# SZU-Speech/Acoustic-Echo-Cancellation

Measured on NVIDIA B200. Metric: audio_seconds_per_second_stage1_aec, higher is better.
Workload: dtype f32

## Files before the change

acoustic_echo_cancellation_b200/csrc/fft_warp.cuh:

```cuda
#pragma once
#include <cuda_runtime.h>

namespace aec {

__device__ __forceinline__ float2 cadd(float2 a, float2 b) { return make_float2(a.x + b.x, a.y + b.y); }
__device__ __forceinline__ float2 csub(float2 a, float2 b) { return make_float2(a.x - b.x, a.y - b.y); }
__device__ __forceinline__ float2 cmul(float2 a, float2 b) {
    return make_float2(fmaf(-a.y, b.y, a.x * b.x), fmaf(a.y, b.x, a.x * b.y));
}
__device__ __forceinline__ float2 cmulc(float2 a, float2 b) {
    return make_float2(fmaf(a.y, b.y, a.x * b.x), fmaf(a.y, b.x, -(a.x * b.y)));
}
__device__ __forceinline__ float2 cfma(float2 a, float2 b, float2 acc) {
    return make_float2(fmaf(-a.y, b.y, fmaf(a.x, b.x, acc.x)), fmaf(a.y, b.x, fmaf(a.x, b.y, acc.y)));
}
__device__ __forceinline__ float2 cfmac(float2 a, float2 b, float2 acc) {
    return make_float2(fmaf(a.y, b.y, fmaf(a.x, b.x, acc.x)), fmaf(-a.y, b.x, fmaf(a.x, b.y, acc.y)));
}

template <bool INV>
__device__ __forceinline__ void radix4(float2& a, float2& b, float2& c, float2& d) {
    const float2 s0 = cadd(a, c), d0 = csub(a, c);
    const float2 s1 = cadd(b, d), d1 = csub(b, d);
    const float2 r = INV ? make_float2(-d1.y, d1.x) : make_float2(d1.y, -d1.x);
    a = cadd(s0, s1);
    c = csub(s0, s1);
    b = cadd(d0, r);
    d = csub(d0, r);
}

template <int M, bool INV>
__device__ __forceinline__ float2 mul_w16(float2 v) {
    constexpr float C1 = 0.92387953251128673848f;
    constexpr float S1 = 0.38268343236508978178f;
    constexpr float R2 = 0.70710678118654752440f;
    if constexpr (M == 0) return v;
    if constexpr (M == 4) return INV ? make_float2(-v.y, v.x) : make_float2(v.y, -v.x);
    if constexpr (M == 2) {
        return INV ? make_float2(R2 * (v.x - v.y), R2 * (v.x + v.y))
                   : make_float2(R2 * (v.x + v.y), R2 * (v.y - v.x));
    }
    if constexpr (M == 6) {
        return INV ? make_float2(-R2 * (v.x + v.y), R2 * (v.x - v.y))
                   : make_float2(R2 * (v.y - v.x), -R2 * (v.x + v.y));
    }
    constexpr float cr = (M == 1) ? C1 : (M == 3) ? S1 :  -C1;
    constexpr float cif = (M == 1) ? -S1 : (M == 3) ? -C1 :  S1;
    constexpr float ci = INV ? -cif : cif;
    return make_float2(fmaf(-v.y, ci, v.x * cr), fmaf(v.y, cr, v.x * ci));
}

__host__ __device__ constexpr int fft16_index(int p) { return (p >> 2) + 4 * (p & 3); }

template <bool INV>
__device__ __forceinline__ void fft16(float2 (&v)[16]) {
#pragma unroll
    for (int j2 = 0; j2 < 4; ++j2) radix4<INV>(v[j2], v[4 + j2], v[8 + j2], v[12 + j2]);
    v[5] = mul_w16<1, INV>(v[5]);
    v[6] = mul_w16<2, INV>(v[6]);
    v[7] = mul_w16<3, INV>(v[7]);
    v[9] = mul_w16<2, INV>(v[9]);
    v[10] = mul_w16<4, INV>(v[10]);
    v[11] = mul_w16<6, INV>(v[11]);
    v[13] = mul_w16<3, INV>(v[13]);
    v[14] = mul_w16<6, INV>(v[14]);
    v[15] = mul_w16<9, INV>(v[15]);
#pragma unroll
    for (int q1 = 0; q1 < 4; ++q1) radix4<INV>(v[4 * q1], v[4 * q1 + 1], v[4 * q1 + 2], v[4 * q1 + 3]);
}

constexpr int kTilePitch = 272;

template <bool INV>
__device__ __forceinline__ void fft256_halfwarp(float2 (&v)[16], float2* tile, const float2* __restrict__ tw,
                                                int h) {
    fft16<INV>(v);
    float2* row = tile + h * 17;
    const float2* twh = tw + h;
#pragma unroll
    for (int p = 0; p < 16; ++p) {
        const int q = fft16_index(p);
        float2 x = v[p];
        if (q != 0) {
            const float2 w = __ldg(twh + q * 16);
            x = INV ? cmulc(x, w) : cmul(x, w);
        }
        row[q] = x;
    }
    __syncwarp();
    const float2* col = tile + h;
#pragma unroll
    for (int l = 0; l < 16; ++l) v[l] = col[l * 17];
    __syncwarp();
    fft16<INV>(v);
}

struct TwiddleRegs {
    float2 w1, w2, w4, w8;
};

template <bool INV>
__device__ __forceinline__ void fft256_halfwarp_regs(float2 (&v)[16], float2* tile, const TwiddleRegs& t, int h) {
    fft16<INV>(v);
    float2* row = tile + h * 17;
    auto pos = [](int q) constexpr { return ((q & 3) << 2) | (q >> 2); };
    auto tw = [](float2 x, float2 w) { return INV ? cmulc(x, w) : cmul(x, w); };
    row[0] = v[pos(0)];
    row[8] = tw(v[pos(8)], t.w8);
    const float2 w3 = cmul(t.w1, t.w2);
#pragma unroll
    for (int low = 1; low < 8; ++low) {
        const float2 wl = (low == 1) ? t.w1 : (low == 2) ? t.w2 : (low == 3) ? w3 : (low == 4) ? t.w4
                        : (low == 5) ? cmul(t.w1, t.w4) : (low == 6) ? cmul(t.w2, t.w4) : cmul(w3, t.w4);
        row[low] = tw(v[pos(low)], wl);
        row[low + 8] = tw(tw(v[pos(low + 8)], wl), t.w8);
    }
    __syncwarp();
    const float2* col = tile + h;
#pragma unroll
    for (int l = 0; l < 16; ++l) v[l] = col[l * 17];
    __syncwarp();
    fft16<INV>(v);
}

struct TwiddleRegs512 {
    float2 w1, w2, w4, w8;
    float2 wr;
    float sgn;
};

template <bool INV>
__device__ __forceinline__ void fft512_warp_regs(float2 (&v)[16], float2* tile, const TwiddleRegs512& t, int lane) {
    fft16<INV>(v);
    const int h = lane & 15, b = lane >> 4;
    float2* row = tile + b * kTilePitch + h * 17;
    auto pos = [](int q) constexpr { return ((q & 3) << 2) | (q >> 2); };
    auto tw = [](float2 x, float2 w) { return INV ? cmulc(x, w) : cmul(x, w); };
    auto pair_step = [&](float2 x) {
        const float px = __shfl_xor_sync(0xffffffffu, x.x, 16);
        const float py = __shfl_xor_sync(0xffffffffu, x.y, 16);
        return tw(make_float2(fmaf(t.sgn, x.x, px), fmaf(t.sgn, x.y, py)), t.wr);
    };
    row[0] = pair_step(v[pos(0)]);
    row[8] = pair_step(tw(v[pos(8)], t.w8));
    const float2 w3 = cmul(t.w1, t.w2);
#pragma unroll
    for (int low = 1; low < 8; ++low) {
        const float2 wl = (low == 1) ? t.w1 : (low == 2) ? t.w2 : (low == 3) ? w3 : (low == 4) ? t.w4
                        : (low == 5) ? cmul(t.w1, t.w4) : (low == 6) ? cmul(t.w2, t.w4) : cmul(w3, t.w4);
        row[low] = pair_step(tw(v[pos(low)], wl));
        row[low + 8] = pair_step(tw(tw(v[pos(low + 8)], wl), t.w8));
    }
    __syncwarp();
    const float2* col = tile + b * kTilePitch + h;
#pragma unroll
    for (int a = 0; a < 16; ++a) v[a] = col[a * 17];
    __syncwarp();
    fft16<INV>(v);
}

}
```

Before: 7.206 million.

## Restructure fft16 butterflies with fused twiddles and vectorize the shared-memory transpose

The 16-point FFT's second radix-4 stage is rewritten so the internal twiddle multiplications are folded into FMA-based butterflies, using tangent-scaled factors, to cut arithmetic instruction count. The shared-memory transpose becomes a common helper that writes 16-byte float4 pairs with an alternating per-row offset instead of scalar float2 stores. Fewer FLOPs and wider stores are meant to reduce ALU and LSU pressure. Risks include small numerical differences from the reordered arithmetic, and misaligned or bank-conflicting float4 stores if the tile base alignment does not match the offset scheme.

```diff
diff --git a/acoustic_echo_cancellation_b200/csrc/fft_warp.cuh b/acoustic_echo_cancellation_b200/csrc/fft_warp.cuh
--- a/acoustic_echo_cancellation_b200/csrc/fft_warp.cuh
+++ b/acoustic_echo_cancellation_b200/csrc/fft_warp.cuh
@@ -29,69 +29,84 @@
     d = csub(d0, r);
 }
 
-template <int M, bool INV>
-__device__ __forceinline__ float2 mul_w16(float2 v) {
-    constexpr float C1 = 0.92387953251128673848f;
-    constexpr float S1 = 0.38268343236508978178f;
-    constexpr float R2 = 0.70710678118654752440f;
-    if constexpr (M == 0) return v;
-    if constexpr (M == 4) return INV ? make_float2(-v.y, v.x) : make_float2(v.y, -v.x);
-    if constexpr (M == 2) {
-        return INV ? make_float2(R2 * (v.x - v.y), R2 * (v.x + v.y))
-                   : make_float2(R2 * (v.x + v.y), R2 * (v.y - v.x));
-    }
-    if constexpr (M == 6) {
-        return INV ? make_float2(-R2 * (v.x + v.y), R2 * (v.x - v.y))
-                   : make_float2(R2 * (v.y - v.x), -R2 * (v.x + v.y));
-    }
-    constexpr float cr = (M == 1) ? C1 : (M == 3) ? S1 :  -C1;
-    constexpr float cif = (M == 1) ? -S1 : (M == 3) ? -C1 :  S1;
-    constexpr float ci = INV ? -cif : cif;
-    return make_float2(fmaf(-v.y, ci, v.x * cr), fmaf(v.y, cr, v.x * ci));
+template <bool INV>
+__device__ __forceinline__ void radix4_out(float2 s0, float2 d0, float2 s1, float2 d1, float k, float2& a, float2& b,
+                                           float2& c, float2& d) {
+    const float2 r = INV ? make_float2(-d1.y, d1.x) : make_float2(d1.y, -d1.x);
+    a = make_float2(fmaf(k, s1.x, s0.x), fmaf(k, s1.y, s0.y));
+    c = make_float2(fmaf(-k, s1.x, s0.x), fmaf(-k, s1.y, s0.y));
+    b = make_float2(fmaf(k, r.x, d0.x), fmaf(k, r.y, d0.y));
+    d = make_float2(fmaf(-k, r.x, d0.x), fmaf(-k, r.y, d0.y));
 }
 
 __host__ __device__ constexpr int fft16_index(int p) { return (p >> 2) + 4 * (p & 3); }
 
 template <bool INV>
 __device__ __forceinline__ void fft16(float2 (&v)[16]) {
+    constexpr float C1 = 0.92387953251128673848f;
+    constexpr float T1 = 0.41421356237309504880f;
+    constexpr float R2 = 0.70710678118654752440f;
+    constexpr float s = INV ? 1.f : -1.f;
 #pragma unroll
     for (int j2 = 0; j2 < 4; ++j2) radix4<INV>(v[j2], v[4 + j2], v[8 + j2], v[12 + j2]);
-    v[5] = mul_w16<1, INV>(v[5]);
-    v[6] = mul_w16<2, INV>(v[6]);
-    v[7] = mul_w16<3, INV>(v[7]);
-    v[9] = mul_w16<2, INV>(v[9]);
-    v[10] = mul_w16<4, INV>(v[10]);
-    v[11] = mul_w16<6, INV>(v[11]);
-    v[13] = mul_w16<3, INV>(v[13]);
-    v[14] = mul_w16<6, INV>(v[14]);
-    v[15] = mul_w16<9, INV>(v[15]);
-#pragma unroll
-    for (int q1 = 0; q1 < 4; ++q1) radix4<INV>(v[4 * q1], v[4 * q1 + 1], v[4 * q1 + 2], v[4 * q1 + 3]);
+    radix4<INV>(v[0], v[1], v[2], v[3]);
+    {
+        const float2 a = v[4], b = v[5], c = v[6], d = v[7];
+        const float2 u = make_float2(c.x - s * c.y, c.y + s * c.x);
+        const float2 s0 = make_float2(fmaf(R2, u.x, a.x), fmaf(R2, u.y, a.y));
+        const float2 d0 = make_float2(fmaf(-R2, u.x, a.x), fmaf(-R2, u.y, a.y));
+        const float2 ub = make_float2(fmaf(-s * T1, b.y, b.x), fmaf(s * T1, b.x, b.y));
+        const float2 ud = make_float2(fmaf(T1, d.x, -s * d.y), fmaf(T1, d.y, s * d.x));
+        radix4_out<INV>(s0, d0, cadd(ub, ud), csub(ub, ud), C1, v[4], v[5], v[6], v[7]);
+    }
+    {
+        const float2 a = v[8], b = v[9], c = v[10], d = v[11];
+        const float2 rc = make_float2(-s * c.y, s * c.x), rd = make_float2(-s * d.y, s * d.x);
+        const float2 p = cadd(b, rd), m = csub(b, rd);
+        radix4_out<INV>(cadd(a, rc), csub(a, rc), make_float2(p.x - s * p.y, p.y + s * p.x),
+                        make_float2(m.x - s * m.y, m.y + s * m.x), R2, v[8], v[9], v[10], v[11]);
+    }
+    {
+        const float2 a = v[12], b = v[13], c = v[14], d = v[15];
+        const float2 u = make_float2(c.x + s * c.y, c.y - s * c.x);
+        const float2 s0 = make_float2(fmaf(-R2, u.x, a.x), fmaf(-R2, u.y, a.y));
+        const float2 d0 = make_float2(fmaf(R2, u.x, a.x), fmaf(R2, u.y, a.y));
+        const float2 ub = make_float2(fmaf(T1, b.x, -s * b.y), fmaf(T1, b.y, s * b.x));
+        const float2 ud = make_float2(fmaf(-s * T1, d.y, d.x), fmaf(s * T1, d.x, d.y));
+        radix4_out<INV>(s0, d0, csub(ub, ud), cadd(ub, ud), C1, v[12], v[13], v[14], v[15]);
+    }
 }
 
 constexpr int kTilePitch = 272;
+
+__device__ __forceinline__ void transpose16(float2 (&v)[16], float2* tile, int h) {
+    float4* row = reinterpret_cast<float4*>(tile + h * 17 + (h & 1));
+#pragma unroll
+    for (int q = 0; q < 16; q += 2) {
+        const float2 a = v[fft16_index(q)], b = v[fft16_index(q + 1)];
+        row[q / 2] = make_float4(a.x, a.y, b.x, b.y);
+    }
+    __syncwarp();
+    const float2* col = tile + h;
+#pragma unroll
+    for (int l = 0; l < 16; ++l) v[l] = col[l * 17 + (l & 1)];
+    __syncwarp();
+}
 
 template <bool INV>
 __device__ __forceinline__ void fft256_halfwarp(float2 (&v)[16], float2* tile, const float2* __restrict__ tw,
                                                 int h) {
     fft16<INV>(v);
-    float2* row = tile + h * 17;
     const float2* twh = tw + h;
 #pragma unroll
     for (int p = 0; p < 16; ++p) {
         const int q = fft16_index(p);
-        float2 x = v[p];
         if (q != 0) {
             const float2 w = __ldg(twh + q * 16);
-            x = INV ? cmulc(x, w) : cmul(x, w);
+            v[p] = INV ? cmulc(v[p], w) : cmul(v[p], w);
         }
-        row[q] = x;
     }
-    __syncwarp();
-    const float2* col = tile + h;
-#pragma unroll
-    for (int l = 0; l < 16; ++l) v[l] = col[l * 17];
-    __syncwarp();
+    transpose16(v, tile, h);
     fft16<INV>(v);
 }
 
@@ -102,24 +117,18 @@
 template <bool INV>
 __device__ __forceinline__ void fft256_halfwarp_regs(float2 (&v)[16], float2* tile, const TwiddleRegs& t, int h) {
     fft16<INV>(v);
-    float2* row = tile + h * 17;
-    auto pos = [](int q) constexpr { return ((q & 3) << 2) | (q >> 2); };
+    auto pos = [](int q) constexpr { return fft16_index(q); };
     auto tw = [](float2 x, float2 w) { return INV ? cmulc(x, w) : cmul(x, w); };
-    row[0] = v[pos(0)];
-    row[8] = tw(v[pos(8)], t.w8);
+    v[pos(8)] = tw(v[pos(8)], t.w8);
     const float2 w3 = cmul(t.w1, t.w2);
 #pragma unroll
     for (int low = 1; low < 8; ++low) {
         const float2 wl = (low == 1) ? t.w1 : (low == 2) ? t.w2 : (low == 3) ? w3 : (low == 4) ? t.w4
                         : (low == 5) ? cmul(t.w1, t.w4) : (low == 6) ? cmul(t.w2, t.w4) : cmul(w3, t.w4);
-        row[low] = tw(v[pos(low)], wl);
-        row[low + 8] = tw(tw(v[pos(low + 8)], wl), t.w8);
+        v[pos(low)] = tw(v[pos(low)], wl);
+        v[pos(low + 8)] = tw(tw(v[pos(low + 8)], wl), t.w8);
     }
-    __syncwarp();
-    const float2* col = tile + h;
-#pragma unroll
-    for (int l = 0; l < 16; ++l) v[l] = col[l * 17];
-    __syncwarp();
+    transpose16(v, tile, h);
     fft16<INV>(v);
 }
 
@@ -133,29 +142,24 @@
 __device__ __forceinline__ void fft512_warp_regs(float2 (&v)[16], float2* tile, const TwiddleRegs512& t, int lane) {
     fft16<INV>(v);
     const int h = lane & 15, b = lane >> 4;
-    float2* row = tile + b * kTilePitch + h * 17;
-    auto pos = [](int q) constexpr { return ((q & 3) << 2) | (q >> 2); };
+    auto pos = [](int q) constexpr { return fft16_index(q); };
     auto tw = [](float2 x, float2 w) { return INV ? cmulc(x, w) : cmul(x, w); };
     auto pair_step = [&](float2 x) {
         const float px = __shfl_xor_sync(0xffffffffu, x.x, 16);
         const float py = __shfl_xor_sync(0xffffffffu, x.y, 16);
         return tw(make_float2(fmaf(t.sgn, x.x, px), fmaf(t.sgn, x.y, py)), t.wr);
     };
-    row[0] = pair_step(v[pos(0)]);
-    row[8] = pair_step(tw(v[pos(8)], t.w8));
+    v[pos(0)] = pair_step(v[pos(0)]);
+    v[pos(8)] = pair_step(tw(v[pos(8)], t.w8));
     const float2 w3 = cmul(t.w1, t.w2);
 #pragma unroll
     for (int low = 1; low < 8; ++low) {
         const float2 wl = (low == 1) ? t.w1 : (low == 2) ? t.w2 : (low == 3) ? w3 : (low == 4) ? t.w4
                         : (low == 5) ? cmul(t.w1, t.w4) : (low == 6) ? cmul(t.w2, t.w4) : cmul(w3, t.w4);
-        row[low] = pair_step(tw(v[pos(low)], wl));
-        row[low + 8] = pair_step(tw(tw(v[pos(low + 8)], wl), t.w8));
+        v[pos(low)] = pair_step(tw(v[pos(low)], wl));
+        v[pos(low + 8)] = pair_step(tw(tw(v[pos(low + 8)], wl), t.w8));
     }
-    __syncwarp();
-    const float2* col = tile + b * kTilePitch + h;
-#pragma unroll
-    for (int a = 0; a < 16; ++a) v[a] = col[a * 17];
-    __syncwarp();
+    transpose16(v, tile + b * kTilePitch, h);
     fft16<INV>(v);
 }
 
```

After: 7.167 million, median of 6. Within noise of the previous version (-0.5%).
